# Hiroshiba/realtime-yukarin

Hardware: NVIDIA H100
Metric: chunks_per_s_0.3s_24kHz_encode_stage1_stage2_vocode (higher is better)
Workload: dtype f64 (WORLD analysis / synthesis, SPTK), f16 operands / f32 accumulate: stage-2 k4 layers on wgmma, stage-1 k4 layers on mma.sync inside the one-launch cluster kernel; f32 CUDA cores (3x3 / k3 edge layers)

## Files before the change

realtime_yukarin_b200/csrc/session.cu:

```cuda
#include <math.h>
#include <stdlib.h>
#include <string.h>
#include <algorithm>
#include <array>
#include <numeric>
#include <vector>

#include "../../include/ryk.h"
#include "engine.h"
#include "features.h"
#include "synth.h"
#include "unet.h"

namespace ryk {

constexpr int kRing = 8;

struct StageGraph {
  cudaGraphExec_t exec = nullptr; long long launches = 0;
  StageGraph() = default;
  StageGraph(const StageGraph&) = delete;
  StageGraph& operator=(const StageGraph&) = delete;
  ~StageGraph() { reset(); }
  void reset() { if (exec) cudaGraphExecDestroy(exec); exec = nullptr; launches = 0; }
};
struct ParityGraphs {
  StageGraph gate;
  StageGraph analysis;
  StageGraph s1_head;
  StageGraph s1;
  StageGraph s2_pro;
  StageGraph s2_layers;
  StageGraph s2_epi;
  StageGraph dec_slide;
  StageGraph synth;
};
struct StepEvents {
  cudaEvent_t gate = nullptr;
  cudaEvent_t enc = nullptr;
  cudaEvent_t cslide = nullptr;
  cudaEvent_t s1 = nullptr;
  cudaEvent_t pro = nullptr;
  cudaEvent_t conv = nullptr;
  cudaEvent_t dslide = nullptr;
  cudaEvent_t dec = nullptr;
  std::array<cudaEvent_t*, 8> all() { return {&gate, &enc, &cslide, &s1, &pro, &conv, &dslide, &dec}; }
};
struct Group;
struct Session {
  cudaEvent_t tev[5][2][kRing]; bool stage_times = false;
  int s1_owner = 0, s2_owner[2] = {0, 0};
  float* d_colmin[2] = {nullptr, nullptr};
  Group* group = nullptr; int slot = 0;
  Voice* voice = nullptr; int voice_id = 0;
  ryk_session_config cfg;
  SptkMats sptk;
  int hop, rate, n_wave, n_feat, e_wave, e_enc_frames, e_conv, e_dec;
  int Lw, Tw, Td, nb, C;
  int Tp;
  long long step = 0;
  long long collected = 0;
  cudaStream_t sE = nullptr, sC = nullptr, sD = nullptr;
  cudaStream_t sC2s[2] = {nullptr, nullptr};
  cudaStream_t sA[2] = {nullptr, nullptr};
  cudaStream_t sA_side = nullptr;
  std::array<cudaStream_t, 7> streams() const { return {sE, sA[0], sA[1], sC, sC2s[0], sC2s[1], sD}; }
  StepEvents ev[kRing];
  float* wave_win[2];
  float *cw_f0[2], *cw_ap[2], *cw_mc[2], *cw_wave[2]; uint8_t* cw_voiced[2];
  float *dw_f0[2], *dw_ap[2], *dw_sp[2];
  float *enc_f0[2], *enc_sp[2], *enc_ap[2], *enc_mc[2]; uint8_t* enc_voiced[2];
  double* d_mse; uint8_t* d_mask[2]; int* d_index[2]; int* d_count[2];
  float *cv_mc_out[2], *cv_f0_out[2], *cv_ap_out[2], *cv_sp_out[2]; uint8_t* cv_voiced_out[2];
  float* cv_sp_mid[2];
  double* dec_f0_f64;
  int max_blocks;
  float* d_chunk[kRing]; float* h_in[kRing];
  double* d_out[kRing]; double* h_out[kRing];
  int* d_n_out[kRing]; int* h_n[kRing];
  float* d_chunk_fixed = nullptr;
  double* d_out_fixed[2];
  int* d_n_fixed[2];
  ParityGraphs graphs[2];
  Synth* synth = nullptr;
  DioPlan* dio[2] = {nullptr, nullptr};
  CrepePlan* crepe[2] = {nullptr, nullptr};
  struct RateSide {
    int rate = 0, up = 1, down = 1, n_taps = 0;
    int hist = 0;
    double* d_h = nullptr;
    ResampleState* d_st = nullptr;
  } in, out;
  int n_in = 0;
  int delay_in = 0;
  int max_out = 0;
  float* in_win[2] = {nullptr, nullptr};
  float* d_chunk_model = nullptr;
  double* out_hist[2] = {nullptr, nullptr};
  double* d_rout_fixed[2] = {nullptr, nullptr}; int* d_rn_fixed[2] = {nullptr, nullptr};
  std::vector<void*> allocs, pinned;
};

struct Group {
  std::vector<Session*> members;
  std::vector<Voice*> voices;
  int owner = 0;
  UNetPlan* p2 = nullptr;
  cudaStream_t sG = nullptr;
  cudaEvent_t ev_fwd[kRing] = {};
  long long step = 0, collected = 0;
  StageGraph fwd_graph;
};

template <typename T>
__global__ void k_slide(const T* __restrict__ old_, const T* __restrict__ new_, T* __restrict__ dst, size_t L, size_t shift, size_t row) {
  size_t total = L * row;
  for (size_t i = blockIdx.x * (size_t)blockDim.x + threadIdx.x; i < total; i += (size_t)gridDim.x * blockDim.x) {
    size_t r = i / row;
    dst[i] = r + shift < L ? old_[i + shift * row] : new_[i - (L - shift) * row];
  }
}

struct SlideDesc { const void* old_; const void* new_; void* dst; size_t L, shift, row; int elem; };
struct SlideBatch { SlideDesc d[5]; int n; };
__global__ void k_slide_multi(SlideBatch b) {
  const SlideDesc& d = b.d[blockIdx.y];
  size_t total = d.L * d.row;
  for (size_t i = blockIdx.x * (size_t)blockDim.x + threadIdx.x; i < total; i += (size_t)gridDim.x * blockDim.x) {
    size_t r = i / d.row;
    bool keep = r + d.shift < d.L;
    size_t src = keep ? i + d.shift * d.row : i - (d.L - d.shift) * d.row;
    if (d.elem == 4) ((uint32_t*)d.dst)[i] = keep ? ((const uint32_t*)d.old_)[src] : ((const uint32_t*)d.new_)[src];
    else ((uint8_t*)d.dst)[i] = keep ? ((const uint8_t*)d.old_)[src] : ((const uint8_t*)d.new_)[src];
  }
}

// ... 62 lines not shown
  if (n > max_samples) n = max_samples;
  for (int i = blockIdx.x * blockDim.x + threadIdx.x; i < n; i += gridDim.x * blockDim.x) { double v = y[i]; if (v != v) y[i] = 0.0; }
  if (blockIdx.x == 0 && threadIdx.x == 0) *n_out = n;
}

template <typename T>
static int slide(const T* old_, const T* new_, T* dst, size_t L, size_t shift, size_t row, cudaStream_t st) {
  size_t total = L * row;
  if (total == 0) return 0;
  int blocks = (int)((total + 255) / 256); if (blocks > 2368) blocks = 2368;
  k_slide<T><<<blocks, 256, 0, st>>>(old_, new_, dst, L, shift, row);
  RYK_CUDA(cudaGetLastError());
  return 0;
}

static int slide_batch(SlideBatch& b, cudaStream_t st) {
  size_t mx = 0;
  for (int i = 0; i < b.n; ++i) { size_t t = b.d[i].L * b.d[i].row; if (t > mx) mx = t; }
  if (mx == 0) return 0;
  int blocks = (int)((mx + 255) / 256); if (blocks > 592) blocks = 592;
  k_slide_multi<<<dim3(blocks, b.n), 256, 0, st>>>(b);
  RYK_CUDA(cudaGetLastError());
  return 0;
}
template <typename T>
static void slide_add(SlideBatch& b, const T* old_, const T* new_, T* dst, size_t L, size_t shift, size_t row) {
  SlideDesc& d = b.d[b.n++];
  d.old_ = old_; d.new_ = new_; d.dst = dst; d.L = L; d.shift = shift; d.row = row; d.elem = (int)sizeof(T);
}

static Session* get_session(Engine* e, int id) { return (id >= 0 && id < (int)e->sessions.size()) ? e->sessions[id] : nullptr; }

static void session_free(Session* s) {
  if (!s) return;
  for (cudaStream_t st : s->streams()) if (st) { cudaStreamSynchronize(st); cudaStreamDestroy(st); }
  if (s->sA_side) cudaStreamDestroy(s->sA_side);
  for (StepEvents& ev : s->ev)
    for (cudaEvent_t* p : ev.all()) if (*p) cudaEventDestroy(*p);
  if (s->stage_times) for (int a = 0; a < 5; ++a) for (int w = 0; w < 2; ++w) for (int i = 0; i < kRing; ++i) cudaEventDestroy(s->tev[a][w][i]);
  for (void* p : s->allocs) cudaFree(p);
  for (void* p : s->pinned) cudaFreeHost(p);
  for (DioPlan* p : s->dio) dio_plan_free(p);
  for (CrepePlan* p : s->crepe) crepe_plan_free(p);
  synth_destroy(s->synth);
  delete s;
}

static void group_free(Group* G) {
  if (!G) return;
  if (G->sG) { cudaStreamSynchronize(G->sG); cudaStreamDestroy(G->sG); }
  for (int i = 0; i < kRing; ++i) if (G->ev_fwd[i]) cudaEventDestroy(G->ev_fwd[i]);
  for (Session* m : G->members) {
    m->group = nullptr;
    for (ParityGraphs& pg : m->graphs) {
      pg.s2_pro.reset();
      pg.s2_epi.reset();
    }
  }
  delete G;
}

void session_destroy_all(Engine* e) {
  for (Reblock* R : e->reblocks) reblock_free(R);
  e->reblocks.clear();
  for (Group* G : e->groups) group_free(G);
  e->groups.clear();
  for (Session* s : e->sessions) session_free(s);
  e->sessions.clear();
}

int session_streams_fork(Engine* e, cudaEvent_t ev) {
  for (Session* s : e->sessions) {
    if (!s) continue;
    for (cudaStream_t st : s->streams()) RYK_CUDA(cudaStreamWaitEvent(st, ev, 0));
  }
  for (Group* G : e->groups) if (G) RYK_CUDA(cudaStreamWaitEvent(G->sG, ev, 0));
  return 0;
}
int session_streams_join(Engine* e) {
  for (Session* s : e->sessions) {
    if (!s) continue;
    for (cudaStream_t st : s->streams()) {
      cudaEvent_t ev;
      RYK_CUDA(cudaEventCreateWithFlags(&ev, cudaEventDisableTiming));
      RYK_CUDA(cudaEventRecord(ev, st));
      RYK_CUDA(cudaStreamWaitEvent(e->stream, ev, 0));
      RYK_CUDA(cudaEventDestroy(ev));
    }
  }
  for (Group* G : e->groups) {
    if (!G) continue;
    cudaEvent_t ev;
    RYK_CUDA(cudaEventCreateWithFlags(&ev, cudaEventDisableTiming));
    RYK_CUDA(cudaEventRecord(ev, G->sG));
    RYK_CUDA(cudaStreamWaitEvent(e->stream, ev, 0));
    RYK_CUDA(cudaEventDestroy(ev));
  }
  return 0;
}


static int graph_kernels(cudaGraph_t graph) {
  size_t n = 0;
  RYK_CUDA(cudaGraphGetNodes(graph, nullptr, &n));
  std::vector<cudaGraphNode_t> nodes(n);
  RYK_CUDA(cudaGraphGetNodes(graph, nodes.data(), &n));
  int kernels = 0;
  for (cudaGraphNode_t node : nodes) {
    cudaGraphNodeType type;
    if (cudaGraphNodeGetType(node, &type) != cudaSuccess) {
      (void)cudaGetLastError();
      continue;
    }
    kernels += type == cudaGraphNodeTypeKernel;
  }
  return kernels;
}

static int stage_graph_init(StageGraph& g, cudaGraph_t graph) {
  const int kernels = graph_kernels(graph);
  if (kernels < 0) return -1;
  RYK_CUDA(cudaGraphInstantiate(&g.exec, graph, 0));
  RYK_CUDA(cudaGraphDestroy(graph));
  g.launches = kernels;
  return 0;
}

static int stage_graph_launch(Engine* e, const StageGraph& g, cudaStream_t st) {
  RYK_CUDA(cudaGraphLaunch(g.exec, st));
  e->launches += g.launches;
  return 0;
}

template <typename F>
static int run_graph(Engine* e, StageGraph& g, cudaStream_t st, F&& body) {
  if (!g.exec) {
    cudaGraph_t graph = nullptr;
    RYK_CUDA(cudaStreamBeginCapture(st, cudaStreamCaptureModeThreadLocal));
    int rc = body();
    cudaError_t err = cudaStreamEndCapture(st, &graph);
    if (rc) return rc;
    RYK_CUDA(err);
    if (stage_graph_init(g, graph)) return -1;
  }
  return stage_graph_launch(e, g, st);
}

struct BucketKernels { int n[16]; };

__global__ void k_set_bucket(cudaGraphConditionalHandle handle, const int* __restrict__ count, int n_buckets, BucketKernels kernels,
                             unsigned long long* __restrict__ launches) {
  if (threadIdx.x == 0 && blockIdx.x == 0) {
    int v = count[0] > 0 ? count[1] / 128 : 0;
    if (v < 0 || v >= n_buckets) v = n_buckets - 1;
    cudaGraphSetConditional(handle, (unsigned)v);
    atomicAdd(launches, (unsigned long long)kernels.n[v]);
  }
}

static int stage1_body(Engine* e, Session* s, int b, int tp1);

static int stage1_build_switch(Engine* e, Session* s, int b) {
  const int n_buckets = s->Tp / 128 + 1;
  RYK_CHECK(n_buckets <= 16, "window too long for the stage-1 graph table");
  cudaGraph_t graph = nullptr;
  RYK_CUDA(cudaGraphCreate(&graph, 0));
  cudaGraphConditionalHandle handle;
  RYK_CUDA(cudaGraphConditionalHandleCreate(&handle, graph, 0, cudaGraphCondAssignDefault));
  cudaGraphNode_t set_node = nullptr;
  const int* cnt = s->d_count[b];
  int nb_ = n_buckets;
  BucketKernels kernels = {};
  void* args[5] = {(void*)&handle, (void*)&cnt, (void*)&nb_, (void*)&kernels, (void*)&e->d_launches};
  cudaKernelNodeParams kp = {};
  kp.func = (void*)k_set_bucket; kp.gridDim = dim3(1); kp.blockDim = dim3(32); kp.sharedMemBytes = 0; kp.kernelParams = args; kp.extra = nullptr;
  RYK_CUDA(cudaGraphAddKernelNode(&set_node, graph, nullptr, 0, &kp));
  cudaGraphNodeParams cp = {};
  cp.type = cudaGraphNodeTypeConditional;
  cp.conditional.handle = handle;
  cp.conditional.type = cudaGraphCondTypeSwitch;
  cp.conditional.size = (unsigned)n_buckets;
  cudaGraphNode_t sw = nullptr;
  RYK_CUDA(cudaGraphAddNode(&sw, graph, &set_node, 1, &cp));
  for (int i = 0; i < n_buckets; ++i) {
    cudaGraph_t body = cp.conditional.phGraph_out[i];
    RYK_CUDA(cudaStreamBeginCaptureToGraph(s->sC, body, nullptr, nullptr, 0, cudaStreamCaptureModeThreadLocal));
    int rc = stage1_body(e, s, b, i * 128);
    cudaGraph_t out = nullptr;
    cudaError_t err = cudaStreamEndCapture(s->sC, &out);
    if (rc) return rc;
    RYK_CUDA(err);
    kernels.n[i] = graph_kernels(body);
    if (kernels.n[i] < 0) return -1;
  }
  RYK_CUDA(cudaGraphKernelNodeSetParams(set_node, &kp));
  return stage_graph_init(s->graphs[b].s1, graph);
}

static int stage1_head(Engine* e, Session* s, int b) {
  const int f = b, g = b ^ 1, pe = s->e_enc_frames;
  const ryk_session_config& c = s->cfg;
  SlideBatch sb; sb.n = 0;
  slide_add<float>(sb, s->cw_f0[f], s->enc_f0[b] + pe, s->cw_f0[g], s->Tw, s->n_feat, 1);
  slide_add<float>(sb, s->cw_ap[f], s->enc_ap[b] + (size_t)pe * s->nb, s->cw_ap[g], s->Tw, s->n_feat, s->nb);
  slide_add<float>(sb, s->cw_mc[f], s->enc_mc[b] + (size_t)pe * s->C, s->cw_mc[g], s->Tw, s->n_feat, s->C);
  slide_add<uint8_t>(sb, s->cw_voiced[f], s->enc_voiced[b] + pe, s->cw_voiced[g], s->Tw, s->n_feat, 1);
  if (slide_batch(sb, s->sC)) return -1;
  return gate_mask_run(e, s->cw_wave[g], s->Tw * s->hop, c.fft_length, s->hop, c.threshold_db, s->Tw, s->d_mse, s->d_mask[b], s->d_index[b],
                       s->d_count[b], s->sC);
}

static int stage1_body(Engine* e, Session* s, int b, int tp1) {
  const int g = b ^ 1;
  const ryk_session_config& c = s->cfg;
  const float* d_y = nullptr;
  if (tp1 > 0) {
    UNetPlan* p1 = nullptr;
    if (unet_get_plan(e, s->voice->stage1, 1, 1, tp1, e->precision, &p1, s->s1_owner)) return -1;
    if (stage1_prologue_run(s->voice, s->cw_mc[g], s->d_index[b], s->d_count[b], s->C, (float*)p1->d_in, tp1, s->sC)) return -1;
    if (unet_forward(e, p1, s->sC)) return -1;
    d_y = (const float*)p1->d_out;
  }
  if (stage1_epilogue_run(s->voice, d_y, s->d_index[b], s->d_mask[b], s->d_count[b], s->Tw, s->C, s->cw_f0[g], s->cw_ap[g], s->cw_voiced[g], s->nb,
                          kSilentMc0, s->cv_mc_out[b], s->cv_f0_out[b], s->cv_ap_out[b], s->cv_voiced_out[b], s->sC)) return -1;
  return mc2sp_run(e, s->sptk.d_H, s->cv_mc_out[b], s->Tw, c.order, c.fft_length, 1e-16, s->cv_sp_mid[b], nullptr, s->sC);
}


static cudaStream_t s2_stream(const Session* s, int b) { return s->sC2s[s->group ? 0 : b]; }
static int s2_plan(Engine* e, const Session* s, int b, UNetPlan** p2) {
  return unet_get_plan(e, s->voice->stage2, 1, s->Tp, 512, e->precision, p2, s->s2_owner[b], s->e_conv, s->n_feat, false, s->Tw);
}

static int stage_time(Session* s, int stage, int which, int r, cudaStream_t st) {
  if (s->stage_times) RYK_CUDA(cudaEventRecord(s->tev[stage][which][r], st));
  return 0;
}

static int session_front(Engine* e, Session* s, const float* d_chunk_user) {
  const long long k = s->step;
  const int b = (int)(k & 1), f = b, g = b ^ 1, r = (int)(k % kRing);
  const ryk_session_config& c = s->cfg;
  const int pe = s->e_enc_frames;
  cudaStream_t sC2 = s2_stream(s, b);
  float* d_colmin = s->d_colmin[s->group ? 0 : b];
  ParityGraphs& pg = s->graphs[b];

  RYK_CUDA(cudaMemcpyAsync(s->d_chunk_fixed, d_chunk_user, sizeof(float) * s->n_in, cudaMemcpyDeviceToDevice, s->sE));
  if (k >= 2) {
    RYK_CUDA(cudaStreamWaitEvent(s->sE, s->ev[(k - 2) % kRing].cslide, 0));
    RYK_CUDA(cudaStreamWaitEvent(s->sE, s->ev[(k - 2) % kRing].enc, 0));
  }
  if (stage_time(s, 0, 0, r, s->sE)) return -1;
  if (run_graph(e, pg.gate, s->sE, [&]() -> int {
        const float* chunk = s->d_chunk_fixed;
        if (s->in.rate) {
          if (slide<float>(s->in_win[f], s->d_chunk_fixed, s->in_win[g], s->in.hist, s->n_in, 1, s->sE)) return -1;
          if (resample_stream_in_run(e, s->in_win[g], s->in.hist, s->n_in, s->delay_in, s->in.up, s->in.down, s->in.d_h, s->in.n_taps,
                                     s->in.d_st + f, s->in.d_st + g, s->d_chunk_model, s->n_wave, s->sE)) return -1;
          chunk = s->d_chunk_model;
        }
        if (slide<float>(s->wave_win[f], chunk, s->wave_win[g], s->Lw, s->n_wave, 1, s->sE)) return -1;
        return slide<float>(s->cw_wave[f], s->wave_win[g] + (size_t)pe * s->hop, s->cw_wave[g], (size_t)s->Tw * s->hop, (size_t)s->n_feat * s->hop, 1, s->sE);
      })) return -1;
  if (stage_time(s, 0, 1, r, s->sE)) return -1;
  RYK_CUDA(cudaEventRecord(s->ev[r].gate, s->sE));

  cudaStream_t sA = s->sA[b];
  RYK_CUDA(cudaStreamWaitEvent(sA, s->ev[r].gate, 0));
  if (k >= 2) RYK_CUDA(cudaStreamWaitEvent(sA, s->ev[(k - 2) % kRing].cslide, 0));
  if (stage_time(s, 1, 0, r, sA)) return -1;
  if (run_graph(e, pg.analysis, sA, [&]() -> int {
        const double* d_f0 = nullptr;
        if (s->crepe[b]) {
          if (crepe_plan_run(e, s->crepe[b], s->wave_win[g], sA)) return -1;
          d_f0 = crepe_plan_f0(s->crepe[b]);
        } else {
          if (dio_stonemask_run(e, s->dio[b], s->wave_win[g], sA)) return -1;
          d_f0 = dio_plan_f0(s->dio[b]);
        }
        const int n_enc = s->Lw / s->hop;
        return spectral_analysis_run(e, s->wave_win[g], s->Lw, c.fs, c.frame_period_ms, d_f0, n_enc, c.fft_length, c.order, s->sptk.d_G,
                                     s->enc_sp[b], s->enc_ap[b], s->enc_mc[b], s->enc_f0[b], s->enc_voiced[b], sA, s->sA_side);
      })) return -1;
  if (stage_time(s, 1, 1, r, sA)) return -1;
  RYK_CUDA(cudaEventRecord(s->ev[r].enc, sA));

  RYK_CUDA(cudaStreamWaitEvent(s->sC, s->ev[r].enc, 0));
  if (stage_time(s, 2, 0, r, s->sC)) return -1;
  if (run_graph(e, pg.s1_head, s->sC, [&]() -> int { return stage1_head(e, s, b); })) return -1;
  RYK_CUDA(cudaEventRecord(s->ev[r].cslide, s->sC));
  if (k >= 2) {
    RYK_CUDA(cudaStreamWaitEvent(s->sC, s->ev[(k - 2) % kRing].dslide, 0));
    RYK_CUDA(cudaStreamWaitEvent(s->sC, s->ev[(k - 2) % kRing].conv, 0));
  }
  if (stage_graph_launch(e, pg.s1, s->sC)) return -1;
  if (stage_time(s, 2, 1, r, s->sC)) return -1;
  RYK_CUDA(cudaEventRecord(s->ev[r].s1, s->sC));

  RYK_CUDA(cudaStreamWaitEvent(sC2, s->ev[r].s1, 0));
  if (k >= 2) RYK_CUDA(cudaStreamWaitEvent(sC2, s->ev[(k - 2) % kRing].dslide, 0));
  if (stage_time(s, 3, 0, r, sC2)) return -1;
  if (s->group) {
    Group* G = s->group;
    if (G->step >= 1) RYK_CUDA(cudaStreamWaitEvent(sC2, G->ev_fwd[(G->step - 1) % kRing], 0));
    float* dst = (float*)G->p2->d_in + (size_t)s->slot * s->Tp * 512;
    if (run_graph(e, pg.s2_pro, sC2, [&]() -> int { return sr_prologue_run(e, s->cv_sp_mid[b], s->Tw, s->Tp, s->nb, dst, sC2, d_colmin); })) return -1;
    RYK_CUDA(cudaEventRecord(s->ev[r].pro, sC2));
  } else {
    UNetPlan* p2 = nullptr;
    if (s2_plan(e, s, b, &p2)) return -1;
    if (run_graph(e, pg.s2_pro, sC2, [&]() -> int {
          if (sr_prologue_run(e, s->cv_sp_mid[b], s->Tw, s->Tp, s->nb, (float*)p2->d_in, sC2, d_colmin)) return -1;
          return unet_forward(e, p2, sC2, 0, 0);
        })) return -1;
  }
  return 0;
}

static int session_mid_single(Engine* e, Session* s) {
  const int b = (int)(s->step & 1);
  cudaStream_t sC2 = s2_stream(s, b);
  UNetPlan* p2 = nullptr;
  if (s2_plan(e, s, b, &p2)) return -1;
  cudaEvent_t pe0 = nullptr, pe1 = nullptr;
  if (e->profile) { RYK_CUDA(cudaEventCreate(&pe0)); RYK_CUDA(cudaEventCreate(&pe1)); RYK_CUDA(cudaEventRecord(pe0, sC2)); }
  if (run_graph(e, s->graphs[b].s2_layers, sC2, [&]() -> int { return unet_forward(e, p2, sC2, 1, 14); })) return -1;
  if (e->profile) { RYK_CUDA(cudaEventRecord(pe1, sC2)); e->prof_events.emplace_back(pe0, pe1); }
  return 0;
}

static int session_back(Engine* e, Session* s) {
  const long long k = s->step;
  const int b = (int)(k & 1), f = b, g = b ^ 1, r = (int)(k % kRing);
  const ryk_session_config& c = s->cfg;
  const int pc = s->e_conv;
  cudaStream_t sC2 = s2_stream(s, b);
  ParityGraphs& pg = s->graphs[b];
  if (s->group) {
    Group* G = s->group;
    RYK_CUDA(cudaStreamWaitEvent(sC2, G->ev_fwd[G->step % kRing], 0));
    const float* src = (const float*)G->p2->d_out + (size_t)s->slot * s->Tp * 512;
    if (run_graph(e, pg.s2_epi, sC2, [&]() -> int { return sr_epilogue_run(e, src, s->Tw, s->nb, s->cv_sp_out[b], sC2, pc, pc + s->n_feat); })) return -1;
  } else {
    UNetPlan* p2 = nullptr;
    if (s2_plan(e, s, b, &p2)) return -1;
    if (run_graph(e, pg.s2_epi, sC2, [&]() -> int {
          if (unet_forward(e, p2, sC2, 15, 15)) return -1;
          return sr_epilogue_run(e, (const float*)p2->d_out, s->Tw, s->nb, s->cv_sp_out[b], sC2, pc, pc + s->n_feat);
        })) return -1;
  }
  if (stage_time(s, 3, 1, r, sC2)) return -1;
  RYK_CUDA(cudaEventRecord(s->ev[r].conv, sC2));

  RYK_CUDA(cudaStreamWaitEvent(s->sD, s->ev[r].conv, 0));
  if (stage_time(s, 4, 0, r, s->sD)) return -1;
  if (synth_host_advance(e, s->synth, s->Td, s->sD)) return -1;
  const int max_blocks = s->max_blocks;
  if (run_graph(e, pg.dec_slide, s->sD, [&]() -> int {
        SlideBatch sb; sb.n = 0;
        slide_add<float>(sb, s->dw_f0[f], s->cv_f0_out[b] + pc, s->dw_f0[g], s->Td, s->n_feat, 1);
        slide_add<float>(sb, s->dw_ap[f], s->cv_ap_out[b] + (size_t)pc * s->nb, s->dw_ap[g], s->Td, s->n_feat, s->nb);
        slide_add<float>(sb, s->dw_sp[f], s->cv_sp_out[b] + (size_t)pc * s->nb, s->dw_sp[g], s->Td, s->n_feat, s->nb);
        if (slide_batch(sb, s->sD)) return -1;
        k_f32_to_f64<<<(s->Td + 127) / 128, 128, 0, s->sD>>>(s->dw_f0[g], s->dec_f0_f64, s->Td);
        RYK_CUDA(cudaGetLastError());
        return 0;
      })) return -1;
  RYK_CUDA(cudaEventRecord(s->ev[r].dslide, s->sD));
  if (run_graph(e, pg.synth, s->sD, [&]() -> int {
        if (synth_add_kernel(e, s->synth, s->dec_f0_f64, s->Td, s->dw_sp[g], s->dw_ap[g], s->sD)) return -1;
        if (synth_drain_async(e, s->synth, s->d_out_fixed[b], max_blocks, s->sD)) return -1;
        k_scrub<<<8, 256, 0, s->sD>>>(s->d_out_fixed[b], s->synth->dev.state, c.vocoder_buffer_size, max_blocks * c.vocoder_buffer_size, s->d_n_fixed[b]);
        RYK_CUDA(cudaGetLastError());
        if (!s->out.rate) return 0;
        return resample_stream_out_run(e, s->out_hist[f], s->out_hist[g], s->out.hist, s->d_out_fixed[b], s->d_n_fixed[b], s->out.up, s->out.down,
                                       s->out.d_h, s->out.n_taps, s->out.d_st + f, s->out.d_st + g, s->d_rout_fixed[b], s->max_out,
                                       s->d_rn_fixed[b], s->sD);
      })) return -1;
  if (stage_time(s, 4, 1, r, s->sD)) return -1;
  s->step++;
  return 0;
}

static int session_enqueue(Engine* e, Session* s, const float* d_chunk_user) {
  int rc = session_front(e, s, d_chunk_user);
  if (!rc) rc = session_mid_single(e, s);
  if (!rc) rc = session_back(e, s);
  return rc;
}

static int group_enqueue(Engine* e, Group* G, const float* const* d_chunks) {
  const int r = (int)(G->step % kRing);
  for (size_t i = 0; i < G->members.size(); ++i)
    if (session_front(e, G->members[i], d_chunks[i])) return -1;
  for (Session* m : G->members) {
    RYK_CUDA(cudaStreamWaitEvent(G->sG, m->ev[m->step % kRing].pro, 0));
    if (m->step >= 1) RYK_CUDA(cudaStreamWaitEvent(G->sG, m->ev[(m->step - 1) % kRing].conv, 0));
  }
  cudaEvent_t pe0 = nullptr, pe1 = nullptr;
  if (e->profile) { RYK_CUDA(cudaEventCreate(&pe0)); RYK_CUDA(cudaEventCreate(&pe1)); RYK_CUDA(cudaEventRecord(pe0, G->sG)); }
  if (run_graph(e, G->fwd_graph, G->sG, [&]() -> int { return unet_forward(e, G->p2, G->sG, 0, 15); })) return -1;
  if (e->profile) { RYK_CUDA(cudaEventRecord(pe1, G->sG)); e->prof_events.emplace_back(pe0, pe1); }
  RYK_CUDA(cudaEventRecord(G->ev_fwd[r], G->sG));
  for (Session* m : G->members)
    if (session_back(e, m)) return -1;
  G->step++;
  return 0;
}

static int stage_in(Session* s, int r, const float* wave) {
  memcpy(s->h_in[r], wave, sizeof(float) * s->n_in);
  RYK_CUDA(cudaMemcpyAsync(s->d_chunk[r], s->h_in[r], sizeof(float) * s->n_in, cudaMemcpyHostToDevice, s->sE));
  return 0;
}

// ... 70 lines not shown
  s->n_feat = (int)lrint(cfg->buffer_time * s->rate);
  s->e_wave = (int)lrint(cfg->encode_extra_time * cfg->fs);
  s->e_enc_frames = (int)lrint(cfg->encode_extra_time * s->rate);
  s->e_conv = (int)lrint(cfg->convert_extra_time * s->rate);
  s->e_dec = (int)lrint(cfg->decode_extra_time * s->rate);
  s->Lw = s->n_wave + 2 * s->e_wave;
  s->Tw = s->n_feat + 2 * s->e_conv;
  s->Td = s->n_feat + 2 * s->e_dec;
  s->Tp = s->Tw + (128 - s->Tw % 128);
  s->nb = cfg->fft_length / 2 + 1;
  s->C = cfg->order + 1;
  RYK_CHECK(s->n_wave == s->n_feat * s->hop && s->e_wave == s->e_enc_frames * s->hop, "buffer_time / encode_extra_time must be whole frames");
  RYK_CHECK(s->Lw / s->hop - 2 * s->e_enc_frames == s->n_feat, "encode window does not trim to one chunk of frames");
  RYK_CHECK(s->nb == 513 && s->voice->stage1->in_ch == s->C, "session configuration does not match the loaded models");
  RYK_CHECK(cheaptrick_fft_size(cfg->fs, 71.0) / 2 + 1 == s->nb,
            "fs does not match fft_length: the synthesizer at this fs needs a different spectrum width (run the session at the model's "
            "rate and set a device rate with ryk_session_set_input_rate / ryk_session_set_output_rate)");
  s->n_in = s->n_wave;
  if (sptk_prepare(e, cfg->order, cfg->alpha, cfg->fft_length, &s->sptk)) return -1;
  int prio_lo = 0, prio_hi = 0;
  RYK_CUDA(cudaDeviceGetStreamPriorityRange(&prio_lo, &prio_hi));
  RYK_CUDA(cudaStreamCreateWithPriority(&s->sE, cudaStreamNonBlocking, prio_hi));
  for (int i = 0; i < 2; ++i) RYK_CUDA(cudaStreamCreateWithPriority(&s->sA[i], cudaStreamNonBlocking, prio_hi));
  RYK_CUDA(cudaStreamCreateWithPriority(&s->sA_side, cudaStreamNonBlocking, prio_hi));
  RYK_CUDA(cudaStreamCreateWithPriority(&s->sC, cudaStreamNonBlocking, prio_hi));
  for (int i = 0; i < 2; ++i) RYK_CUDA(cudaStreamCreateWithPriority(&s->sC2s[i], cudaStreamNonBlocking, prio_lo));
  RYK_CUDA(cudaStreamCreateWithPriority(&s->sD, cudaStreamNonBlocking, prio_hi));
  for (StepEvents& ev : s->ev)
    for (cudaEvent_t* p : ev.all()) RYK_CUDA(cudaEventCreateWithFlags(p, cudaEventDisableTiming));
  { const char* v = getenv("RYK_STAGE_TIMES"); s->stage_times = v && atoi(v) != 0; }
  if (s->stage_times) for (int a = 0; a < 5; ++a) for (int w = 0; w < 2; ++w) for (int i = 0; i < kRing; ++i) RYK_CUDA(cudaEventCreate(&s->tev[a][w][i]));
  auto A = [&](void** p, size_t bytes) -> int { RYK_CUDA(cudaMalloc(p, bytes ? bytes : 16)); RYK_CUDA(cudaMemsetAsync(*p, 0, bytes ? bytes : 16, e->stream)); s->allocs.push_back(*p); return 0; };
  auto P = [&](void** p, size_t bytes) -> int { RYK_CUDA(cudaMallocHost(p, bytes ? bytes : 16)); memset(*p, 0, bytes ? bytes : 16); s->pinned.push_back(*p); return 0; };
  const int n_enc = s->Lw / s->hop;
  for (int i = 0; i < 2; ++i) {
    if (A((void**)&s->wave_win[i], sizeof(float) * s->Lw)) return -1;
    if (A((void**)&s->cw_f0[i], sizeof(float) * s->Tw)) return -1;
    if (A((void**)&s->cw_ap[i], sizeof(float) * (size_t)s->Tw * s->nb)) return -1;
    if (A((void**)&s->cw_mc[i], sizeof(float) * (size_t)s->Tw * s->C)) return -1;
    if (A((void**)&s->cw_voiced[i], (size_t)s->Tw)) return -1;
    if (A((void**)&s->cw_wave[i], sizeof(float) * (size_t)s->Tw * s->hop)) return -1;
    if (A((void**)&s->dw_f0[i], sizeof(float) * s->Td)) return -1;
    if (A((void**)&s->dw_ap[i], sizeof(float) * (size_t)s->Td * s->nb)) return -1;
    if (A((void**)&s->dw_sp[i], sizeof(float) * (size_t)s->Td * s->nb)) return -1;
    k_fill_rows<float><<<64, 256, 0, e->stream>>>(s->cw_mc[i], s->Tw, s->C, kSilentMc0, 0.f);
    if (A((void**)&s->enc_f0[i], sizeof(float) * n_enc)) return -1;
    if (A((void**)&s->enc_sp[i], sizeof(float) * (size_t)n_enc * s->nb)) return -1;
    if (A((void**)&s->enc_ap[i], sizeof(float) * (size_t)n_enc * s->nb)) return -1;
    if (A((void**)&s->enc_mc[i], sizeof(float) * (size_t)n_enc * s->C)) return -1;
    if (A((void**)&s->enc_voiced[i], (size_t)n_enc)) return -1;
    if (A((void**)&s->d_mask[i], (size_t)s->Tw)) return -1;
    if (A((void**)&s->d_index[i], sizeof(int) * s->Tw)) return -1;
    if (A((void**)&s->d_count[i], sizeof(int) * 2)) return -1;
    if (A((void**)&s->cv_mc_out[i], sizeof(float) * (size_t)s->Tw * s->C)) return -1;
    if (A((void**)&s->cv_f0_out[i], sizeof(float) * s->Tw)) return -1;
    if (A((void**)&s->cv_ap_out[i], sizeof(float) * (size_t)s->Tw * s->nb)) return -1;
    if (A((void**)&s->cv_sp_out[i], sizeof(float) * (size_t)s->Tw * s->nb)) return -1;
    if (A((void**)&s->cv_voiced_out[i], (size_t)s->Tw)) return -1;
    if (A((void**)&s->cv_sp_mid[i], sizeof(float) * (size_t)s->Tw * s->nb)) return -1;
  }
  if (A((void**)&s->d_mse, sizeof(double) * s->Tw)) return -1;
  for (int i = 0; i < 2; ++i) if (A((void**)&s->d_colmin[i], sizeof(float) * kColminFloats)) return -1;
  if (A((void**)&s->dec_f0_f64, sizeof(double) * s->Td)) return -1;
  if (A((void**)&s->d_chunk_fixed, sizeof(float) * s->n_wave)) return -1;
  s->max_blocks = (s->Td * s->hop) / cfg->vocoder_buffer_size + 4;
  s->max_out = s->max_blocks * cfg->vocoder_buffer_size;
  const size_t out_samples = (size_t)s->max_out;
  for (int i = 0; i < 2; ++i) {
    if (A((void**)&s->d_out_fixed[i], sizeof(double) * out_samples)) return -1;
    if (A((void**)&s->d_n_fixed[i], sizeof(int))) return -1;
  }
  for (int i = 0; i < kRing; ++i) {
    if (A((void**)&s->d_chunk[i], sizeof(float) * s->n_wave)) return -1;
    if (A((void**)&s->d_out[i], sizeof(double) * out_samples)) return -1;
    if (A((void**)&s->d_n_out[i], sizeof(int))) return -1;
    if (P((void**)&s->h_in[i], sizeof(float) * s->n_wave)) return -1;
    if (P((void**)&s->h_out[i], sizeof(double) * out_samples)) return -1;
    if (P((void**)&s->h_n[i], sizeof(int))) return -1;
  }
  for (int i = 0; i < 2; ++i) {
    const int rc = e->f0_method == 2 ? crepe_plan_create(e, s->Lw, cfg->fs, cfg->frame_period_ms, &s->crepe[i])
                                     : dio_plan_create(e, s->Lw, cfg->fs, cfg->frame_period_ms, cfg->f0_floor, cfg->f0_ceil, &s->dio[i], e->f0_method);
    if (rc) return -1;
  }
  if (synth_create(e, cfg->fs, cfg->frame_period_ms, cheaptrick_fft_size(cfg->fs, 71.0), cfg->vocoder_buffer_size, 4096, &s->synth)) return -1;
  UNetPlan* p = nullptr;
  s->s1_owner = ++e->plan_owners;
  for (int b = 0; b < 2; ++b) s->s2_owner[b] = ++e->plan_owners;
  for (int Tp = 128; Tp <= s->Tp; Tp += 128) if (unet_get_plan(e, s->voice->stage1, 1, 1, Tp, e->precision, &p, s->s1_owner)) return -1;
  RYK_CUDA(cudaStreamSynchronize(e->stream));
  RYK_CUDA(cudaDeviceSynchronize());
  for (int b = 0; b < 2; ++b) if (stage1_build_switch(e, s, b)) return -1;
  return 0;
}

int ryk_session_destroy(ryk_engine* h, int id) {
  Engine* e = &h->impl;
  Session* s = get_session(e, id);
  RYK_CHECK(s != nullptr, "no such session");
  RYK_CHECK(s->group == nullptr, "session belongs to a group: destroy the group first");
  RYK_CUDA(cudaStreamSynchronize(e->stream));
  const int s1_owner = s->s1_owner, s2_owner[2] = {s->s2_owner[0], s->s2_owner[1]};
  Voice* v = s->voice;
  session_free(s);
  unet_release_owner(v->stage1, s1_owner);
  for (int owner : s2_owner) unet_release_owner(v->stage2, owner);
  v->users--;
  e->sessions[id] = nullptr;
  return 0;
}

int ryk_session_submit(ryk_engine* h, int id, const float* wave, int n, long long* ticket) {
  Engine* e = &h->impl;
  RYK_CUDA(cudaSetDevice(e->device));
  Session* s = get_session(e, id);
  RYK_CHECK(s != nullptr, "no such session");
  RYK_CHECK(n == s->n_in, "chunk length must be round(rate * buffer_time) at the session's input rate");
  RYK_CHECK(s->group == nullptr, "session belongs to a group: use ryk_group_submit");
  RYK_CHECK(s->step - s->collected < kRing - 2, "too many chunks in flight: collect before submitting more");
  const long long k = s->step;
  const int r = (int)(k % kRing);
  if (stage_in(s, r, wave)) return -1;
  if (session_enqueue(e, s, s->d_chunk[r])) return -1;
  if (stage_out(s, r, s->h_out[r], s->h_n[r], cudaMemcpyDeviceToHost)) return -1;
  if (ticket) *ticket = k;
  return 0;
}

int ryk_session_collect(ryk_engine* h, int id, long long ticket, double* out, int out_capacity, int* n_out) {
  Engine* e = &h->impl;
  Session* s = get_session(e, id);
  RYK_CHECK(s != nullptr, "no such session");
  RYK_CHECK(ticket == s->collected && ticket < s->step, "tickets are collected in submission order");
  return collect_out(s, ticket, out, out_capacity, n_out);
}

int ryk_session_poll(ryk_engine* h, int id, long long ticket, int* done) {
  Engine* e = &h->impl;
  Session* s = get_session(e, id);
  RYK_CHECK(s != nullptr && done != nullptr, "no such session");
  RYK_CHECK(ticket >= 0 && ticket < s->step && ticket + kRing > s->step, "ticket is not among the last 8 steps");
  cudaError_t q = cudaEventQuery(s->ev[ticket % kRing].dec);
  if (q != cudaSuccess && q != cudaErrorNotReady) RYK_CUDA(q);
  *done = q == cudaSuccess ? 1 : 0;
  return 0;
// ... 117 lines not shown
    if (s->n_in != s0->n_in || s->in.rate != s0->in.rate || s->out.rate != s0->out.rate)
      return "group members must have the same device input and output rates";
  std::vector<const Voice*> voices;
  for (const Session* s : members)
    if (std::find(voices.begin(), voices.end(), s->voice) == voices.end()) voices.push_back(s->voice);
  if (voices.size() > 1 && e->precision != 1) return "a group of several voices needs precision 1 (FP16 tensor cores)";
  if ((int)voices.size() > kMaxGroupVoices) return "a group holds at most 8 distinct voices";
  const UNet* n0 = voices[0]->stage2;
  for (const Voice* v : voices)
    if (v->stage2->in_ch != n0->in_ch || v->stage2->out_ch != n0->out_ch || v->stage2->base != n0->base)
      return "the members' stage-2 models must have the same (in, out, base) channels";
  return nullptr;
}

static bool session_idle(const Session* s) { return s->collected == s->step; }

static int group_rebuild(Engine* e, Group* G, const std::vector<Session*>& members) {
  const char* refusal = group_refusal(e, members);
  if (refusal) { set_error(refusal); return -1; }
  RYK_CUDA(cudaDeviceSynchronize());
  std::vector<Voice*> voices;
  std::vector<int> voice_of;
  for (Session* m : members) {
    const auto it = std::find(voices.begin(), voices.end(), m->voice);
    voice_of.push_back((int)(it - voices.begin()));
    if (it == voices.end()) voices.push_back(m->voice);
  }
  std::vector<const UNet*> nets;
  for (const Voice* v : voices) nets.push_back(v->stage2);
  std::vector<int> kb, kl;
  for (Session* m : members) { kb.push_back(m->e_conv); kl.push_back(m->n_feat); }
  int keep_begin = 0, keep_len = 0;
  keep_hull((int)members.size(), kb.data(), kl.data(), &keep_begin, &keep_len);
  const int owner = ++e->plan_owners;
  UNetPlan* p2 = nullptr;
  if (unet_get_plan(e, voices[0]->stage2, (int)members.size(), members[0]->Tp, 512, e->precision, &p2, owner, keep_begin, keep_len, false,
                    members[0]->Tw) ||
      unet_plan_set_voices(p2, nets, voice_of)) {
    unet_release_owner(voices[0]->stage2, owner);
    return -1;
  }
  if (G->p2) unet_release_owner(G->voices[0]->stage2, G->owner);
  for (Voice* v : G->voices) v->users--;
  for (Voice* v : voices) v->users++;
  G->voices = voices; G->owner = owner; G->p2 = p2;
  G->fwd_graph.reset();
  for (size_t i = 0; i < members.size(); ++i) {
    Session* m = members[i];
    if (m->group != G) {
      for (int b = 0; b < 2; ++b) unet_release_owner(m->voice->stage2, m->s2_owner[b]);
      for (ParityGraphs& pg : m->graphs) pg.s2_layers.reset();
    }
    m->group = G; m->slot = (int)i;
    for (ParityGraphs& pg : m->graphs) { pg.s2_pro.reset(); pg.s2_epi.reset(); }
  }
  G->members = members;
  return 0;
}

int ryk_group_create(ryk_engine* h, const int* session_ids, int n_sessions, int* group_id) {
  Engine* e = &h->impl;
  RYK_CUDA(cudaSetDevice(e->device));
  RYK_CHECK(session_ids && group_id && n_sessions >= 1 && n_sessions <= kMaxGroupBatch, "a group holds 1..64 sessions");
  std::vector<Session*> members;
  for (int i = 0; i < n_sessions; ++i) {
    Session* s = get_session(e, session_ids[i]);
    RYK_CHECK(s && !s->group && std::find(members.begin(), members.end(), s) == members.end(),
              "group members must be distinct sessions with the same window length, none of them in a group");
    RYK_CHECK(session_idle(s), "collect every submitted chunk of a session before it joins a group");
    members.push_back(s);
  }
  Group* G = new Group();
  if (group_rebuild(e, G, members)) { delete G; return -1; }
  { int lo = 0, hi = 0; RYK_CUDA(cudaDeviceGetStreamPriorityRange(&lo, &hi)); RYK_CUDA(cudaStreamCreateWithPriority(&G->sG, cudaStreamNonBlocking, lo)); }
  for (int i = 0; i < kRing; ++i) RYK_CUDA(cudaEventCreateWithFlags(&G->ev_fwd[i], cudaEventDisableTiming));
  RYK_CUDA(cudaDeviceSynchronize());
  e->groups.push_back(G);
  *group_id = (int)e->groups.size() - 1;
  return 0;
}

int ryk_group_add(ryk_engine* h, int group_id, int session_id) {
  Engine* e = &h->impl;
  RYK_CUDA(cudaSetDevice(e->device));
  Group* G = get_group(e, group_id);
  RYK_CHECK(G != nullptr, "no such group");
  Session* s = get_session(e, session_id);
  RYK_CHECK(s != nullptr, "no such session");
  RYK_CHECK(s->group == nullptr, "the session is already in a group");
  RYK_CHECK(G->collected == G->step, "collect every submitted chunk of the group before changing its members");
  RYK_CHECK(session_idle(s), "collect every submitted chunk of a session before it joins a group");
  std::vector<Session*> members = G->members;
  members.push_back(s);
  return group_rebuild(e, G, members);
}

int ryk_group_remove(ryk_engine* h, int group_id, int session_id) {
  Engine* e = &h->impl;
  RYK_CUDA(cudaSetDevice(e->device));
  Group* G = get_group(e, group_id);
  RYK_CHECK(G != nullptr, "no such group");
  Session* s = get_session(e, session_id);
  RYK_CHECK(s != nullptr && s->group == G, "the session is not a member of this group");
  RYK_CHECK(G->members.size() > 1, "the session is the group's last member: destroy the group instead");
  RYK_CHECK(G->collected == G->step, "collect every submitted chunk of the group before changing its members");
  std::vector<Session*> members = G->members;
  members.erase(members.begin() + s->slot);
  RYK_CUDA(cudaDeviceSynchronize());
  for (int b = 0; b < 2; ++b) {
    UNetPlan* p = nullptr;
    if (s2_plan(e, s, b, &p)) {
      for (int c = 0; c < 2; ++c) unet_release_owner(s->voice->stage2, s->s2_owner[c]);
      return -1;
    }
  }
  if (group_rebuild(e, G, members)) {
    for (int b = 0; b < 2; ++b) unet_release_owner(s->voice->stage2, s->s2_owner[b]);
    return -1;
  }
  s->group = nullptr; s->slot = 0;
  for (ParityGraphs& pg : s->graphs) { pg.s2_pro.reset(); pg.s2_layers.reset(); pg.s2_epi.reset(); }
  return 0;
}

int ryk_group_members(ryk_engine* h, int group_id, int* session_ids, int capacity) {
  Engine* e = &h->impl;
  Group* G = get_group(e, group_id);
  RYK_CHECK(G != nullptr, "no such group");
  const int n = (int)G->members.size();
  for (int i = 0; i < n && i < capacity && session_ids; ++i) {
    const auto it = std::find(e->sessions.begin(), e->sessions.end(), G->members[i]);
    session_ids[i] = (int)(it - e->sessions.begin());
  }
  return n;
}

int ryk_group_destroy(ryk_engine* h, int group_id) {
  Engine* e = &h->impl;
  Group* G = get_group(e, group_id);
  RYK_CHECK(G != nullptr, "no such group");
  RYK_CUDA(cudaDeviceSynchronize());
  const int owner = G->owner;
  const std::vector<Voice*> voices = G->voices;
  group_free(G);
  unet_release_owner(voices[0]->stage2, owner);
  for (Voice* v : voices) v->users--;
  e->groups[group_id] = nullptr;
  return 0;
}

int ryk_group_size(ryk_engine* h, int group_id) {
  Group* G = get_group(&h->impl, group_id);
  return G ? (int)G->members.size() : -1;
}

int ryk_group_submit(ryk_engine* h, int group_id, const float* const* waves, int n, long long* ticket) {
  Engine* e = &h->impl;
  RYK_CUDA(cudaSetDevice(e->device));
  Group* G = get_group(e, group_id);
  RYK_CHECK(G != nullptr, "no such group");
  RYK_CHECK(G->step - G->collected < kRing - 2, "too many chunks in flight: collect before submitting more");
  const long long k = G->step;
  const int r = (int)(k % kRing);
  std::vector<const float*> d_chunks(G->members.size());
  for (size_t i = 0; i < G->members.size(); ++i) {
    Session* s = G->members[i];
    RYK_CHECK(n == s->n_in, "chunk length must be round(rate * buffer_time) at the session's input rate");
    if (stage_in(s, r, waves[i])) return -1;
    d_chunks[i] = s->d_chunk[r];
  }
  if (group_enqueue(e, G, d_chunks.data())) return -1;
  for (Session* s : G->members)
    if (stage_out(s, r, s->h_out[r], s->h_n[r], cudaMemcpyDeviceToHost)) return -1;
  if (ticket) *ticket = k;
// ... 187 lines not shown
```

Before: 2298.

## Triple-buffer stage-1 to stage-2 handoff buffers to deepen cross-step pipelining

Converted-feature handoff buffers (cv_*_out, cv_sp_mid) go from two parity slots to three. Stage 1 of step k now waits only on step k-3's decode slide and conversion instead of step k-2's, so an extra step can be in flight. Graphs that touch these buffers are captured per (parity, handoff) combination, six variants, and uploaded ahead of use. The cost is more device memory, more captured graphs and more setup time.

```diff
diff --git a/realtime_yukarin_b200/csrc/session.cu b/realtime_yukarin_b200/csrc/session.cu
--- a/realtime_yukarin_b200/csrc/session.cu
+++ b/realtime_yukarin_b200/csrc/session.cu
@@ -15,6 +15,8 @@
 namespace ryk {
 
 constexpr int kRing = 8;
+constexpr int kHandoff = 3;
+constexpr int kHandoffGraphs = 6;
 
 struct StageGraph {
   cudaGraphExec_t exec = nullptr; long long launches = 0;
@@ -28,12 +30,14 @@
   StageGraph gate;
   StageGraph analysis;
   StageGraph s1_head;
+  StageGraph s2_layers;
+  StageGraph synth;
+};
+struct HandoffGraphs {
   StageGraph s1;
   StageGraph s2_pro;
-  StageGraph s2_layers;
   StageGraph s2_epi;
   StageGraph dec_slide;
-  StageGraph synth;
 };
 struct StepEvents {
   cudaEvent_t gate = nullptr;
@@ -71,8 +75,8 @@
   float *dw_f0[2], *dw_ap[2], *dw_sp[2];
   float *enc_f0[2], *enc_sp[2], *enc_ap[2], *enc_mc[2]; uint8_t* enc_voiced[2];
   double* d_mse; uint8_t* d_mask[2]; int* d_index[2]; int* d_count[2];
-  float *cv_mc_out[2], *cv_f0_out[2], *cv_ap_out[2], *cv_sp_out[2]; uint8_t* cv_voiced_out[2];
-  float* cv_sp_mid[2];
+  float *cv_mc_out[kHandoff], *cv_f0_out[kHandoff], *cv_ap_out[kHandoff], *cv_sp_out[kHandoff]; uint8_t* cv_voiced_out[kHandoff];
+  float* cv_sp_mid[kHandoff];
   double* dec_f0_f64;
   int max_blocks;
   float* d_chunk[kRing]; float* h_in[kRing];
@@ -82,6 +86,7 @@
   double* d_out_fixed[2];
   int* d_n_fixed[2];
   ParityGraphs graphs[2];
+  HandoffGraphs hgraphs[kHandoffGraphs];
   Synth* synth = nullptr;
   DioPlan* dio[2] = {nullptr, nullptr};
   CrepePlan* crepe[2] = {nullptr, nullptr};
@@ -250,9 +255,9 @@
   for (int i = 0; i < kRing; ++i) if (G->ev_fwd[i]) cudaEventDestroy(G->ev_fwd[i]);
   for (Session* m : G->members) {
     m->group = nullptr;
-    for (ParityGraphs& pg : m->graphs) {
-      pg.s2_pro.reset();
-      pg.s2_epi.reset();
+    for (HandoffGraphs& hg : m->hgraphs) {
+      hg.s2_pro.reset();
+      hg.s2_epi.reset();
     }
   }
   delete G;
@@ -331,16 +336,32 @@
 }
 
 template <typename F>
+static int capture_graph(StageGraph& g, cudaStream_t st, F&& body) {
+  cudaGraph_t graph = nullptr;
+  RYK_CUDA(cudaStreamBeginCapture(st, cudaStreamCaptureModeThreadLocal));
+  int rc = body();
+  cudaError_t err = cudaStreamEndCapture(st, &graph);
+  if (rc) return rc;
+  RYK_CUDA(err);
+  return stage_graph_init(g, graph);
+}
+
+template <typename F>
 static int run_graph(Engine* e, StageGraph& g, cudaStream_t st, F&& body) {
-  if (!g.exec) {
-    cudaGraph_t graph = nullptr;
-    RYK_CUDA(cudaStreamBeginCapture(st, cudaStreamCaptureModeThreadLocal));
-    int rc = body();
-    cudaError_t err = cudaStreamEndCapture(st, &graph);
-    if (rc) return rc;
-    RYK_CUDA(err);
-    if (stage_graph_init(g, graph)) return -1;
-  }
+  if (!g.exec && capture_graph(g, st, body)) return -1;
+  return stage_graph_launch(e, g, st);
+}
+
+template <typename F>
+static int run_handoff_graph(Engine* e, Session* s, long long k, StageGraph HandoffGraphs::*which, cudaStream_t st, F&& body) {
+  StageGraph& g = s->hgraphs[k % kHandoffGraphs].*which;
+  if (!g.exec)
+    for (int j = (int)(k & 1); j < kHandoffGraphs; j += 2) {
+      StageGraph& gj = s->hgraphs[j].*which;
+      if (gj.exec) continue;
+      if (capture_graph(gj, st, [&]() -> int { return body(j % kHandoff); })) return -1;
+      if (&gj != &g) RYK_CUDA(cudaGraphUpload(gj.exec, st));
+    }
   return stage_graph_launch(e, g, st);
 }
 
@@ -356,9 +377,10 @@
   }
 }
 
-static int stage1_body(Engine* e, Session* s, int b, int tp1);
-
-static int stage1_build_switch(Engine* e, Session* s, int b) {
+static int stage1_body(Engine* e, Session* s, int b, int h, int tp1);
+
+static int stage1_build_switch(Engine* e, Session* s, int j) {
+  const int b = j & 1, h = j % kHandoff;
   const int n_buckets = s->Tp / 128 + 1;
   RYK_CHECK(n_buckets <= 16, "window too long for the stage-1 graph table");
   cudaGraph_t graph = nullptr;
@@ -383,7 +405,7 @@
   for (int i = 0; i < n_buckets; ++i) {
     cudaGraph_t body = cp.conditional.phGraph_out[i];
     RYK_CUDA(cudaStreamBeginCaptureToGraph(s->sC, body, nullptr, nullptr, 0, cudaStreamCaptureModeThreadLocal));
-    int rc = stage1_body(e, s, b, i * 128);
+    int rc = stage1_body(e, s, b, h, i * 128);
     cudaGraph_t out = nullptr;
     cudaError_t err = cudaStreamEndCapture(s->sC, &out);
     if (rc) return rc;
@@ -392,7 +414,9 @@
     if (kernels.n[i] < 0) return -1;
   }
   RYK_CUDA(cudaGraphKernelNodeSetParams(set_node, &kp));
-  return stage_graph_init(s->graphs[b].s1, graph);
+  if (stage_graph_init(s->hgraphs[j].s1, graph)) return -1;
+  RYK_CUDA(cudaGraphUpload(s->hgraphs[j].s1.exec, s->sC));
+  return 0;
 }
 
 static int stage1_head(Engine* e, Session* s, int b) {
@@ -408,7 +432,7 @@
                        s->d_count[b], s->sC);
 }
 
-static int stage1_body(Engine* e, Session* s, int b, int tp1) {
+static int stage1_body(Engine* e, Session* s, int b, int h, int tp1) {
   const int g = b ^ 1;
   const ryk_session_config& c = s->cfg;
   const float* d_y = nullptr;
@@ -420,8 +444,8 @@
     d_y = (const float*)p1->d_out;
   }
   if (stage1_epilogue_run(s->voice, d_y, s->d_index[b], s->d_mask[b], s->d_count[b], s->Tw, s->C, s->cw_f0[g], s->cw_ap[g], s->cw_voiced[g], s->nb,
-                          kSilentMc0, s->cv_mc_out[b], s->cv_f0_out[b], s->cv_ap_out[b], s->cv_voiced_out[b], s->sC)) return -1;
-  return mc2sp_run(e, s->sptk.d_H, s->cv_mc_out[b], s->Tw, c.order, c.fft_length, 1e-16, s->cv_sp_mid[b], nullptr, s->sC);
+                          kSilentMc0, s->cv_mc_out[h], s->cv_f0_out[h], s->cv_ap_out[h], s->cv_voiced_out[h], s->sC)) return -1;
+  return mc2sp_run(e, s->sptk.d_H, s->cv_mc_out[h], s->Tw, c.order, c.fft_length, 1e-16, s->cv_sp_mid[h], nullptr, s->sC);
 }
 
 
@@ -488,28 +512,30 @@
   if (stage_time(s, 2, 0, r, s->sC)) return -1;
   if (run_graph(e, pg.s1_head, s->sC, [&]() -> int { return stage1_head(e, s, b); })) return -1;
   RYK_CUDA(cudaEventRecord(s->ev[r].cslide, s->sC));
-  if (k >= 2) {
-    RYK_CUDA(cudaStreamWaitEvent(s->sC, s->ev[(k - 2) % kRing].dslide, 0));
-    RYK_CUDA(cudaStreamWaitEvent(s->sC, s->ev[(k - 2) % kRing].conv, 0));
-  }
-  if (stage_graph_launch(e, pg.s1, s->sC)) return -1;
+  if (k >= kHandoff) {
+    RYK_CUDA(cudaStreamWaitEvent(s->sC, s->ev[(k - 3) % kRing].dslide, 0));
+    RYK_CUDA(cudaStreamWaitEvent(s->sC, s->ev[(k - 3) % kRing].conv, 0));
+  }
+  if (stage_graph_launch(e, s->hgraphs[k % kHandoffGraphs].s1, s->sC)) return -1;
   if (stage_time(s, 2, 1, r, s->sC)) return -1;
   RYK_CUDA(cudaEventRecord(s->ev[r].s1, s->sC));
 
   RYK_CUDA(cudaStreamWaitEvent(sC2, s->ev[r].s1, 0));
-  if (k >= 2) RYK_CUDA(cudaStreamWaitEvent(sC2, s->ev[(k - 2) % kRing].dslide, 0));
+  if (k >= kHandoff) RYK_CUDA(cudaStreamWaitEvent(sC2, s->ev[(k - 3) % kRing].dslide, 0));
   if (stage_time(s, 3, 0, r, sC2)) return -1;
   if (s->group) {
     Group* G = s->group;
     if (G->step >= 1) RYK_CUDA(cudaStreamWaitEvent(sC2, G->ev_fwd[(G->step - 1) % kRing], 0));
     float* dst = (float*)G->p2->d_in + (size_t)s->slot * s->Tp * 512;
-    if (run_graph(e, pg.s2_pro, sC2, [&]() -> int { return sr_prologue_run(e, s->cv_sp_mid[b], s->Tw, s->Tp, s->nb, dst, sC2, d_colmin); })) return -1;
+    if (run_handoff_graph(e, s, k, &HandoffGraphs::s2_pro, sC2, [&](int h) -> int {
+          return sr_prologue_run(e, s->cv_sp_mid[h], s->Tw, s->Tp, s->nb, dst, sC2, d_colmin);
+        })) return -1;
     RYK_CUDA(cudaEventRecord(s->ev[r].pro, sC2));
   } else {
     UNetPlan* p2 = nullptr;
     if (s2_plan(e, s, b, &p2)) return -1;
-    if (run_graph(e, pg.s2_pro, sC2, [&]() -> int {
-          if (sr_prologue_run(e, s->cv_sp_mid[b], s->Tw, s->Tp, s->nb, (float*)p2->d_in, sC2, d_colmin)) return -1;
+    if (run_handoff_graph(e, s, k, &HandoffGraphs::s2_pro, sC2, [&](int h) -> int {
+          if (sr_prologue_run(e, s->cv_sp_mid[h], s->Tw, s->Tp, s->nb, (float*)p2->d_in, sC2, d_colmin)) return -1;
           return unet_forward(e, p2, sC2, 0, 0);
         })) return -1;
   }
@@ -539,13 +565,15 @@
     Group* G = s->group;
     RYK_CUDA(cudaStreamWaitEvent(sC2, G->ev_fwd[G->step % kRing], 0));
     const float* src = (const float*)G->p2->d_out + (size_t)s->slot * s->Tp * 512;
-    if (run_graph(e, pg.s2_epi, sC2, [&]() -> int { return sr_epilogue_run(e, src, s->Tw, s->nb, s->cv_sp_out[b], sC2, pc, pc + s->n_feat); })) return -1;
+    if (run_handoff_graph(e, s, k, &HandoffGraphs::s2_epi, sC2, [&](int h) -> int {
+          return sr_epilogue_run(e, src, s->Tw, s->nb, s->cv_sp_out[h], sC2, pc, pc + s->n_feat);
+        })) return -1;
   } else {
     UNetPlan* p2 = nullptr;
     if (s2_plan(e, s, b, &p2)) return -1;
-    if (run_graph(e, pg.s2_epi, sC2, [&]() -> int {
+    if (run_handoff_graph(e, s, k, &HandoffGraphs::s2_epi, sC2, [&](int h) -> int {
           if (unet_forward(e, p2, sC2, 15, 15)) return -1;
-          return sr_epilogue_run(e, (const float*)p2->d_out, s->Tw, s->nb, s->cv_sp_out[b], sC2, pc, pc + s->n_feat);
+          return sr_epilogue_run(e, (const float*)p2->d_out, s->Tw, s->nb, s->cv_sp_out[h], sC2, pc, pc + s->n_feat);
         })) return -1;
   }
   if (stage_time(s, 3, 1, r, sC2)) return -1;
@@ -555,11 +583,11 @@
   if (stage_time(s, 4, 0, r, s->sD)) return -1;
   if (synth_host_advance(e, s->synth, s->Td, s->sD)) return -1;
   const int max_blocks = s->max_blocks;
-  if (run_graph(e, pg.dec_slide, s->sD, [&]() -> int {
+  if (run_handoff_graph(e, s, k, &HandoffGraphs::dec_slide, s->sD, [&](int h) -> int {
         SlideBatch sb; sb.n = 0;
-        slide_add<float>(sb, s->dw_f0[f], s->cv_f0_out[b] + pc, s->dw_f0[g], s->Td, s->n_feat, 1);
-        slide_add<float>(sb, s->dw_ap[f], s->cv_ap_out[b] + (size_t)pc * s->nb, s->dw_ap[g], s->Td, s->n_feat, s->nb);
-        slide_add<float>(sb, s->dw_sp[f], s->cv_sp_out[b] + (size_t)pc * s->nb, s->dw_sp[g], s->Td, s->n_feat, s->nb);
+        slide_add<float>(sb, s->dw_f0[f], s->cv_f0_out[h] + pc, s->dw_f0[g], s->Td, s->n_feat, 1);
+        slide_add<float>(sb, s->dw_ap[f], s->cv_ap_out[h] + (size_t)pc * s->nb, s->dw_ap[g], s->Td, s->n_feat, s->nb);
+        slide_add<float>(sb, s->dw_sp[f], s->cv_sp_out[h] + (size_t)pc * s->nb, s->dw_sp[g], s->Td, s->n_feat, s->nb);
         if (slide_batch(sb, s->sD)) return -1;
         k_f32_to_f64<<<(s->Td + 127) / 128, 128, 0, s->sD>>>(s->dw_f0[g], s->dec_f0_f64, s->Td);
         RYK_CUDA(cudaGetLastError());
@@ -736,6 +764,8 @@
     if (A((void**)&s->d_mask[i], (size_t)s->Tw)) return -1;
     if (A((void**)&s->d_index[i], sizeof(int) * s->Tw)) return -1;
     if (A((void**)&s->d_count[i], sizeof(int) * 2)) return -1;
+  }
+  for (int i = 0; i < kHandoff; ++i) {
     if (A((void**)&s->cv_mc_out[i], sizeof(float) * (size_t)s->Tw * s->C)) return -1;
     if (A((void**)&s->cv_f0_out[i], sizeof(float) * s->Tw)) return -1;
     if (A((void**)&s->cv_ap_out[i], sizeof(float) * (size_t)s->Tw * s->nb)) return -1;
@@ -774,7 +804,7 @@
   for (int Tp = 128; Tp <= s->Tp; Tp += 128) if (unet_get_plan(e, s->voice->stage1, 1, 1, Tp, e->precision, &p, s->s1_owner)) return -1;
   RYK_CUDA(cudaStreamSynchronize(e->stream));
   RYK_CUDA(cudaDeviceSynchronize());
-  for (int b = 0; b < 2; ++b) if (stage1_build_switch(e, s, b)) return -1;
+  for (int j = 0; j < kHandoffGraphs; ++j) if (stage1_build_switch(e, s, j)) return -1;
   return 0;
 }
 
@@ -998,7 +1028,7 @@
       for (ParityGraphs& pg : m->graphs) pg.s2_layers.reset();
     }
     m->group = G; m->slot = (int)i;
-    for (ParityGraphs& pg : m->graphs) { pg.s2_pro.reset(); pg.s2_epi.reset(); }
+    for (HandoffGraphs& hg : m->hgraphs) { hg.s2_pro.reset(); hg.s2_epi.reset(); }
   }
   G->members = members;
   return 0;
@@ -1065,7 +1095,8 @@
     return -1;
   }
   s->group = nullptr; s->slot = 0;
-  for (ParityGraphs& pg : s->graphs) { pg.s2_pro.reset(); pg.s2_layers.reset(); pg.s2_epi.reset(); }
+  for (ParityGraphs& pg : s->graphs) pg.s2_layers.reset();
+  for (HandoffGraphs& hg : s->hgraphs) { hg.s2_pro.reset(); hg.s2_epi.reset(); }
   return 0;
 }
 
```

Result: faster. 2507, median of 6 (+9.1%).
